# JoeyT1994/TensorNetworkQuantumSimulator.jl

Measured on AMD Instinct MI355X. Metric: two-site gates/sec at fixed chi (LxL TFIM Trotter layer), higher is better.
Workload: dtype c64 (ComplexF32; Gram/eigen steps in f64; the chi = 32 plane products as exact bf16 x 3 splits with f32 accumulation, TNQS_NO_BF16X3=1 for f32 matrix instructions)

## Files before the change

### include/tnqs_debug.h

```cpp
#ifndef TNQS_DEBUG_H
#define TNQS_DEBUG_H
#include <stdint.h>
#include "tnqs.h"
#ifdef __cplusplus
extern "C" {
#endif
int tnqs_dbg_jacobi(int dtype, int m, int n, void* A_inout, void* V_out, int* sweeps_out);
int tnqs_dbg_theta_svd_pre(int m, int n, int nq, void* A_inout, const void* Q, void* V_out, int* sweeps_out, int copies, int reps, double* ms_out, double* phase_us_out ,
                           int cap );
int tnqs_dbg_time_jacobi_f32(int m, int n, const void* A, int copies, int reps, double* ms_out, int* sweeps_out);
int tnqs_dbg_chol(int n, const void* G, void* L_out, void* W_out, int* fail_out, double tau);
int tnqs_dbg_fiber_gemm(int dtype, int D, int PA, int K, int PB, int Do, int No, const void* in, const void* X, void* out,
                        double* norm2_out, int use_mfma);
int tnqs_dbg_gram(int dtype, int D, int PA, int K, int PB, const void* X, const void* Y, void* out, int acc64, int use_mfma);
int tnqs_dbg_gram_fused(int PA, int K, int PB, const void* X, const void* Y, const void* M, void* out);
int tnqs_dbg_gauge_gram(int z, const int* chi, int bleg, const void* X, const void* M, void* out);
int tnqs_dbg_pair(int C0, int NMID, int NHI, const void* in, const void* Mx, const void* My, void* out);
int tnqs_dbg_pair_legs(int d, int z, const int* chi, int lx, int ly, const void* in, const void* Mx, const void* My, void* out);
int tnqs_dbg_pair_gram(int d, int z, const int* chi, int lx, int ly, const void* X, const void* Y, const void* M, void* out);
int tnqs_dbg_pair_gram2(int d, int z, const int* chi, int lx, int ly, const void* X, const void* Y, const void* Mx, const void* My, void* out_y, void* out_x);
int tnqs_dbg_bench_plane(int which, int nsites, int lx, int ly, int reps, double* ms);
#define TNQS_DBG_ROUTE_X3 1
#define TNQS_DBG_ROUTE_F32 2
#define TNQS_DBG_ROUTE_F64 3
#define TNQS_DBG_ROUTE_F64_SHARED 4
#define TNQS_DBG_ROUTE_HALF_LINES 5
#define TNQS_DBG_ROUTE_WHOLE_LINES 6
#define TNQS_DBG_ROUTE_SMALL_SCALAR 7
#define TNQS_DBG_ROUTE_SMALL_MFMA16 8
int tnqs_dbg_rowgemm(int D, int K, int nitems, const int* PA, const int* PB, const int* No, const void* in, const void* X, void* out, double* norm2_out,
                     int tpw, int* route_out);
int tnqs_dbg_gram_mfma(int nitems, const int* shape, const void* X, const void* Y, void* out, int nchunks, int* route_out);
int tnqs_dbg_pair16(int d, int nitems, const int* z, const int* chi, const int* lx, const int* ly, const void* in, const void* M, void* out, int spw, int* route_out);
int tnqs_dbg_pair_gram2x16(int d, int nitems, const int* z, const int* chi, const int* lx, const int* ly, const int* both, const void* X, const void* Y, const void* M,
                           void* out_y, void* out_x, int spw);
int tnqs_dbg_svd_tall(int nitems, const int* m, const int* n, void* A, int* chol_fail, int* polished, int* sweeps);
int tnqs_dbg_small_site(int nitems, const int* d, const int* z, const int* chi, const int* jo, const void* psi, const void* M, const int* present, int form,
                        const void* old_msg, const int* has_old, int normalize, void* out, void* new_msg, double* diff_out, int* route_out);
int tnqs_dbg_msg_finalize(int dtype, int nitems, const int* chi, const int* nchunks, const void* partials, const void* old_msg, const int* has_old, int normalize,
                          void* new_msg, double* diff_out);
int tnqs_dbg_default_sequence(tnqs_handle h, int* src, int* dst, int cap, int* n_out);
int tnqs_dbg_default_sequence_graph(int nv, int ne, const int32_t* esrc, const int32_t* edst, int* src, int* dst, int* level, int cap, int* n_out);
int tnqs_dbg_gate_schedule(int nv, int ne, const int32_t* esrc, const int32_t* edst, int ngates, const int32_t* nverts, const int32_t* verts, int update_cache,
                           int* step_of_gate, int* step_is_bp, int cap, int* nsteps_out);
#ifdef __cplusplus
}
#endif
#endif
```

### profiles/plane_bench.py

```python
import ctypes as C
import os
import sys

here = os.path.dirname(os.path.abspath(__file__))
lib = C.CDLL(os.path.join(here, "..", "tensornetworkquantumsimulator.jl_amd", "libtnqs_hip.so"))
lib.tnqs_dbg_bench_plane.argtypes = [C.c_int, C.c_int, C.c_int, C.c_int, C.c_int, C.POINTER(C.c_double)]
nsites = int(sys.argv[1]) if len(sys.argv) > 1 else 100
reps = int(sys.argv[2]) if len(sys.argv) > 2 else 5
n = 2 * 32 ** 4
for which, name, flops in ((0, "pair", 2 * 8.0 * n * 32), (1, "pair_gram2", 4 * 8.0 * n * 32)):
    for lx, ly in ((0, 1), (0, 2), (0, 3), (1, 2), (1, 3), (2, 3)):
        ms = C.c_double(0)
        rc = lib.tnqs_dbg_bench_plane(which, nsites, lx, ly, reps, C.byref(ms))
        if rc != 0:
            print(name, (lx, ly), "rc", rc)
            continue
        print(f"{name:11s} legs ({lx},{ly})  {ms.value:8.3f} ms  {flops * nsites / ms.value / 1e9:7.1f} TFLOP/s")
```

### tensornetworkquantumsimulator.jl_amd/csrc/api.cpp

```cpp
#include <cmath>
#include <cstring>
#include <string>
#include "engine.hpp"

using namespace tnqs;

struct tnqs_state_s { State* s; };

static thread_local std::string g_err;

template <class F> static int guard(F&& f) {
    try { f(); return TNQS_OK; }
    catch (const Err& e) { g_err = e.what(); return e.code; }
    catch (const std::bad_alloc&) { g_err = "out of host memory"; return TNQS_ERR_HIP; }
    catch (const std::exception& e) { g_err = e.what(); return TNQS_ERR_INVALID; }
    catch (...) { g_err = "unknown error"; return TNQS_ERR_INVALID; }
}
static State* S(tnqs_handle h) { if (!h || !h->s) throw Err(TNQS_ERR_INVALID, "null handle"); return h->s; }

extern "C" {

int tnqs_version(void) { return 102; }
const char* tnqs_last_error(void) { return g_err.c_str(); }
int tnqs_device_count(int* count) {
// ... 138 lines not shown

int tnqs_profile_enable(tnqs_handle h, int on) { return guard([&] { S(h)->prof->on = on != 0; }); }
int tnqs_profile_get(tnqs_handle h, int cls, int64_t* launches, double* ms, double* bytes, double* flops) {
    return guard([&] {
        State* s = S(h);
        if (cls < 0 || cls >= TNQS_PROF_NCLASSES) throw Err(TNQS_ERR_INVALID, "profile_get: bad class");
        prof_collect(s);
        const ProfClass& pc = s->prof->cls[cls];
        if (launches) *launches = pc.launches;
        if (ms) *ms = pc.ms;
        if (bytes) *bytes = pc.bytes;
        if (flops) *flops = pc.flops;
    });
}
int tnqs_profile_reset(tnqs_handle h) {
    return guard([&] { State* s = S(h); prof_collect(s); for (auto& p : s->prof->cls) p = ProfClass{}; });
}

}

#include "../../include/tnqs_debug.h"
#include "kernels.hpp"
namespace tnqs { void dbg_default_sequence(const Graph& g, std::vector<int>& src, std::vector<int>& dst);
                 std::shared_ptr<Graph> dbg_make_graph(int nv, int ne, const int32_t* es, const int32_t* ed);
                 void dbg_default_sequence_graph(const Graph& g, std::vector<int>& src, std::vector<int>& dst, std::vector<int>& level);
                 void dbg_pair(int C0, int NMID, int NHI, const void* in, const void* Mx, const void* My, void* out);
                 void dbg_gram_fused(int PA, int K, int PB, const void* X, const void* Y, const void* M, void* out);
                 void dbg_gauge_gram(int z, const int* chi, int bleg, const void* X, const void* M, void* out);
                 void dbg_jacobi(int dtype, int m, int n, void* A, void* V, int* sweeps);
                 void dbg_chol(int n, const void* G, void* L, void* W, int* fail, double tau);
                 void dbg_theta_svd_pre(int m, int n, int nq, void* A, const void* Q, void* V, int* sweeps, int copies, int reps, double* ms, double* phase_us, int cap);
                 void dbg_time_jacobi_f32(int m, int n, const void* A, int copies, int reps, double* ms, int* sweeps);
                 void dbg_pair_legs(int d, int z, const int* chi, int lx, int ly, const void* in, const void* Mx, const void* My, void* out);
                 void dbg_pair_gram2(int d, int z, const int* chi, int lx, int ly, const void* X, const void* Y, const void* Mx, const void* My, void* out_y, void* out_x);
                 void dbg_bench_plane(int which, int nsites, int lx, int ly, int reps, double* ms);
                 void dbg_pair_gram(int d, int z, const int* chi, int lx, int ly, const void* X, const void* Y, const void* M, void* out);
                 void dbg_fiber_gemm(int dtype, int D, int PA, int K, int PB, int Do, int No, const void* in, const void* X, void* out, double* norm2, int use_mfma);
                 void dbg_gram(int dtype, int D, int PA, int K, int PB, const void* X, const void* Y, void* out, int acc64, int use_mfma);
                 void dbg_rowgemm(int D, int K, int nitems, const int* PA, const int* PB, const int* No, const void* in, const void* X, void* out, double* norm2, int tpw, int* route);
                 void dbg_gram_mfma(int nitems, const int* shape, const void* X, const void* Y, void* out, int nchunks, int* route);
                 void dbg_pair16(int d, int nitems, const int* z, const int* chi, const int* lx, const int* ly, const void* in, const void* M, void* out, int spw, int* route);
                 void dbg_pair_gram2x16(int d, int nitems, const int* z, const int* chi, const int* lx, const int* ly, const int* both, const void* X, const void* Y, const void* M,
                                        void* out_y, void* out_x, int spw);
                 void dbg_svd_tall(int nitems, const int* m, const int* n, void* A, int* chol_fail, int* polished, int* sweeps);
                 void dbg_small_site(int nitems, const int* d, const int* z, const int* chi, const int* jo, const void* psi, const void* M, const int* present, int form,
                                     const void* old_msg, const int* has_old, int normalize, void* out, void* new_msg, double* diff, int* route);
                 void dbg_msg_finalize(int dtype, int nitems, const int* chi, const int* nchunks, const void* partials, const void* old_msg, const int* has_old, int normalize,
                                       void* new_msg, double* diff); }
extern "C" {
int tnqs_dbg_default_sequence(tnqs_handle h, int* src, int* dst, int cap, int* n_out) {
    return guard([&] { std::vector<int> a, b; dbg_default_sequence(*S(h)->g, a, b); *n_out = (int)a.size();
                       for (int i = 0; i < (int)a.size() && i < cap; ++i) { src[i] = a[i]; dst[i] = b[i]; } });
}
int tnqs_dbg_default_sequence_graph(int nv, int ne, const int32_t* esrc, const int32_t* edst, int* src, int* dst, int* level, int cap, int* n_out) {
    return guard([&] { if (nv < 0 || ne < 0 || (ne > 0 && (!esrc || !edst)) || !n_out) throw Err(TNQS_ERR_INVALID, "tnqs_dbg_default_sequence_graph: bad arguments");
                       auto g = dbg_make_graph(nv, ne, esrc, edst); std::vector<int> a, b, l; dbg_default_sequence_graph(*g, a, b, l); *n_out = (int)a.size();
                       for (int i = 0; i < (int)a.size() && i < cap; ++i) { if (src) src[i] = a[i]; if (dst) dst[i] = b[i]; if (level) level[i] = l[i]; } });
}
int tnqs_dbg_gate_schedule(int nv, int ne, const int32_t* esrc, const int32_t* edst, int ngates, const int32_t* nverts, const int32_t* verts, int update_cache,
                           int* step_of_gate, int* step_is_bp, int cap, int* nsteps_out) {
    return guard([&] { if (nv < 0 || ne < 0 || (ne > 0 && (!esrc || !edst)) || ngates < 0 || (ngates > 0 && (!nverts || !verts)) || !nsteps_out) throw Err(TNQS_ERR_INVALID, "tnqs_dbg_gate_schedule: bad arguments");
                       for (int i = 0, o = 0; i < ngates; o += nverts[i], ++i) { if (nverts[i] < 1 || nverts[i] > 2) throw Err(TNQS_ERR_INVALID, "tnqs_dbg_gate_schedule: only one- and two-site gates");
                                                                                 for (int k = 0; k < nverts[i]; ++k) if (verts[o + k] < 0 || verts[o + k] >= nv) throw Err(TNQS_ERR_INVALID, "tnqs_dbg_gate_schedule: vertex out of range"); }
                       auto g = dbg_make_graph(nv, ne, esrc, edst); const GateSchedule steps = build_gate_schedule(*g, ngates, nverts, verts, update_cache != 0); *nsteps_out = (int)steps.size();
                       for (int k = 0; k < (int)steps.size(); ++k) { if (step_is_bp && k < cap) step_is_bp[k] = steps[k].is_bp ? 1 : 0; if (step_of_gate) for (int i = steps[k].begin; i < steps[k].end; ++i) step_of_gate[i] = k; } });
}
int tnqs_dbg_jacobi(int dtype, int m, int n, void* A, void* V, int* sweeps) { return guard([&] { dbg_jacobi(dtype, m, n, A, V, sweeps); }); }
int tnqs_dbg_theta_svd_pre(int m, int n, int nq, void* A, const void* Q, void* V, int* sweeps, int copies, int reps, double* ms, double* phase_us, int cap) { return guard([&] { dbg_theta_svd_pre(m, n, nq, A, Q, V, sweeps, copies, reps, ms, phase_us, cap); }); }
int tnqs_dbg_time_jacobi_f32(int m, int n, const void* A, int copies, int reps, double* ms, int* sweeps) { return guard([&] { dbg_time_jacobi_f32(m, n, A, copies, reps, ms, sweeps); }); }
int tnqs_dbg_chol(int n, const void* G, void* L, void* W, int* fail, double tau) { return guard([&] { dbg_chol(n, G, L, W, fail, tau); }); }
int tnqs_dbg_fiber_gemm(int dtype, int D, int PA, int K, int PB, int Do, int No, const void* in, const void* X, void* out, double* norm2, int use_mfma) {
    return guard([&] { dbg_fiber_gemm(dtype, D, PA, K, PB, Do, No, in, X, out, norm2, use_mfma); });
}
int tnqs_dbg_pair(int C0, int NMID, int NHI, const void* in, const void* Mx, const void* My, void* out) { return guard([&] { dbg_pair(C0, NMID, NHI, in, Mx, My, out); }); }
int tnqs_dbg_pair_legs(int d, int z, const int* chi, int lx, int ly, const void* in, const void* Mx, const void* My, void* out) { return guard([&] { dbg_pair_legs(d, z, chi, lx, ly, in, Mx, My, out); }); }
int tnqs_dbg_pair_gram2(int d, int z, const int* chi, int lx, int ly, const void* X, const void* Y, const void* Mx, const void* My, void* out_y, void* out_x) {
    return guard([&] { dbg_pair_gram2(d, z, chi, lx, ly, X, Y, Mx, My, out_y, out_x); });
}
int tnqs_dbg_bench_plane(int which, int nsites, int lx, int ly, int reps, double* ms) { return guard([&] { dbg_bench_plane(which, nsites, lx, ly, reps, ms); }); }
int tnqs_dbg_pair_gram(int d, int z, const int* chi, int lx, int ly, const void* X, const void* Y, const void* M, void* out) { return guard([&] { dbg_pair_gram(d, z, chi, lx, ly, X, Y, M, out); }); }
int tnqs_dbg_gram_fused(int PA, int K, int PB, const void* X, const void* Y, const void* M, void* out) { return guard([&] { dbg_gram_fused(PA, K, PB, X, Y, M, out); }); }
int tnqs_dbg_gauge_gram(int z, const int* chi, int bleg, const void* X, const void* M, void* out) { return guard([&] { dbg_gauge_gram(z, chi, bleg, X, M, out); }); }
int tnqs_dbg_gram(int dtype, int D, int PA, int K, int PB, const void* X, const void* Y, void* out, int acc64, int use_mfma) {
    return guard([&] { dbg_gram(dtype, D, PA, K, PB, X, Y, out, acc64, use_mfma); });
}
int tnqs_dbg_rowgemm(int D, int K, int nitems, const int* PA, const int* PB, const int* No, const void* in, const void* X, void* out, double* norm2_out, int tpw, int* route_out) {
    return guard([&] { dbg_rowgemm(D, K, nitems, PA, PB, No, in, X, out, norm2_out, tpw, route_out); });
}
int tnqs_dbg_gram_mfma(int nitems, const int* shape, const void* X, const void* Y, void* out, int nchunks, int* route_out) {
    return guard([&] { dbg_gram_mfma(nitems, shape, X, Y, out, nchunks, route_out); });
}
int tnqs_dbg_pair16(int d, int nitems, const int* z, const int* chi, const int* lx, const int* ly, const void* in, const void* M, void* out, int spw, int* route_out) {
    return guard([&] { dbg_pair16(d, nitems, z, chi, lx, ly, in, M, out, spw, route_out); });
}
int tnqs_dbg_pair_gram2x16(int d, int nitems, const int* z, const int* chi, const int* lx, const int* ly, const int* both, const void* X, const void* Y, const void* M,
                           void* out_y, void* out_x, int spw) {
    return guard([&] { dbg_pair_gram2x16(d, nitems, z, chi, lx, ly, both, X, Y, M, out_y, out_x, spw); });
}
int tnqs_dbg_svd_tall(int nitems, const int* m, const int* n, void* A, int* chol_fail, int* polished, int* sweeps) {
    return guard([&] { dbg_svd_tall(nitems, m, n, A, chol_fail, polished, sweeps); });
}
int tnqs_dbg_small_site(int nitems, const int* d, const int* z, const int* chi, const int* jo, const void* psi, const void* M, const int* present, int form,
                        const void* old_msg, const int* has_old, int normalize, void* out, void* new_msg, double* diff_out, int* route_out) {
    return guard([&] { dbg_small_site(nitems, d, z, chi, jo, psi, M, present, form, old_msg, has_old, normalize, out, new_msg, diff_out, route_out); });
}
int tnqs_dbg_msg_finalize(int dtype, int nitems, const int* chi, const int* nchunks, const void* partials, const void* old_msg, const int* has_old, int normalize,
                          void* new_msg, double* diff_out) {
    return guard([&] { dbg_msg_finalize(dtype, nitems, chi, nchunks, partials, old_msg, has_old, normalize, new_msg, diff_out); });
// ... 3 lines not shown
```

### tensornetworkquantumsimulator.jl_amd/csrc/debug.cpp

```cpp
#include <cstdio>
#include <cstring>
#include <cstdlib>
#include <vector>
#include <algorithm>
#include <memory>
#include <string>
#include "engine.hpp"
#include "kernels.hpp"
#include "launch_util.hpp"
#include "../../include/tnqs_debug.h"

namespace tnqs {
#define HIPCHK(x) hipchk((x), #x)
struct DBuf { void* p = nullptr; explicit DBuf(size_t n) { HIPCHK(hipMalloc(&p, n ? n : 1)); } ~DBuf() { (void)hipFree(p); }
              void up(const void* h, size_t n) { HIPCHK(hipMemcpy(p, h, n, hipMemcpyHostToDevice)); } void down(void* h, size_t n) { HIPCHK(hipMemcpy(h, p, n, hipMemcpyDeviceToHost)); } };
static void need_gpu() { int n = 0; if (hipGetDeviceCount(&n) != hipSuccess || n <= 0) throw Err(TNQS_ERR_HIP, "no HIP device available"); }

void dbg_jacobi(int dtype, int m, int n, void* A, void* V, int* sweeps) {
    need_gpu();
    if (m < 1 || n < 1 || m > 256 || n > 256) throw Err(TNQS_ERR_INVALID, "dbg_jacobi: 1 <= m, n <= 256");
    size_t esz = dtype == TNQS_C64 ? 8 : 16;
    DBuf dA((size_t)m * n * esz), dV((size_t)n * n * esz), dS(4), dI(sizeof(JacobiItem));
    dA.up(A, (size_t)m * n * esz);
    if (dtype == TNQS_C64) launch_identity<float>(nullptr, dV.p, n); else launch_identity<double>(nullptr, dV.p, n);
// ... 152 lines not shown
}
void dbg_pair(int C0, int NMID, int NHI, const void* in, const void* Mx, const void* My, void* out) {
    need_gpu();
    if (C0 % 16) throw Err(TNQS_ERR_INVALID, "dbg_pair: C0 % 16 != 0");
    size_t n = (size_t)C0 * 32 * NMID * 32 * NHI;
    DBuf dIn(n * 8), dOut(n * 8), dX(32 * 32 * 8), dY(32 * 32 * 8), dI(sizeof(PairItem));
    dIn.up(in, n * 8); dX.up(Mx, 32 * 32 * 8); dY.up(My, 32 * 32 * 8);
    HIPCHK(hipMemset(dOut.p, 0xff, n * 8));
    PairItem it{}; it.in = dIn.p; it.out = dOut.p; it.Mx = dX.p; it.My = dY.p;
    it.g.cstr = 2; it.g.sx = C0; it.g.sy = (long long)C0 * 32 * NMID; it.g.n0 = C0 / 16; it.g.t0 = 16; it.g.n1 = NMID; it.g.t1 = (long long)C0 * 32;
    it.g.n2 = NHI; it.g.t2 = (long long)C0 * 32 * NMID * 32;
    const int wgs = plan_pair(&it, 1, 3);
    dI.up(&it, sizeof(it));
    launch_mfma_pair(nullptr, (const PairItem*)dI.p, 1, wgs);
    HIPCHK(hipDeviceSynchronize());
    dOut.down(out, n * 8);
}
void dbg_pair_legs(int d, int z, const int* chi, int lx, int ly, const void* in, const void* Mx, const void* My, void* out) {
    need_gpu();
    PairItem it{};
    if (!pair_geometry(d, z, chi, lx, ly, it.g)) throw Err(TNQS_ERR_UNSUPPORTED, "dbg_pair_legs: shape not covered by the pair kernel");
    size_t n = d; for (int i = 0; i < z; ++i) n *= chi[i];
    DBuf dIn(n * 8), dOut(n * 8), dX(32 * 32 * 8), dY(32 * 32 * 8), dI(sizeof(PairItem));
    dIn.up(in, n * 8); dX.up(Mx, 32 * 32 * 8); dY.up(My, 32 * 32 * 8);
    HIPCHK(hipMemset(dOut.p, 0xff, n * 8));
    it.in = dIn.p; it.out = dOut.p; it.Mx = dX.p; it.My = dY.p;
    if ((size_t)it.g.n0 * it.g.n1 * it.g.n2 * 16 * 1024 != n) throw Err(TNQS_ERR_INVALID, "dbg_pair_legs: slice count");
    const int wgs = plan_pair(&it, 1, 3);
    dI.up(&it, sizeof(it));
    launch_mfma_pair(nullptr, (const PairItem*)dI.p, 1, wgs);
    HIPCHK(hipDeviceSynchronize());
    dOut.down(out, n * 8);
}
void dbg_pair_gram(int d, int z, const int* chi, int lx, int ly, const void* X, const void* Y, const void* M, void* out) {
    need_gpu();
    PairGramItem it{};
    if (!pair_geometry(d, z, chi, lx, ly, it.g)) throw Err(TNQS_ERR_UNSUPPORTED, "dbg_pair_gram: shape not covered by the pair kernel");
    size_t n = d; for (int i = 0; i < z; ++i) n *= chi[i];
    const bool x3 = mfma_use_x3();
    PairGram2Item one{}; one.g = it.g;
    const int nwg = x3 ? plan_x3_pair_gram1(&one, 1, nullptr, 3) : plan_pair_gram(&it, 1, nullptr, 3), npart = nwg;
    DBuf dX(n * 8), dY(n * 8), dM(32 * 32 * 8), dI(sizeof(PairGram2Item)), dR(sizeof(ReduceItem)), dP((size_t)npart * 1024 * 8), dO(1024 * 8);
    dX.up(X, n * 8); dY.up(Y, n * 8); dM.up(M, 32 * 32 * 8);
    it.X = dX.p; it.Y = dY.p; it.M = dM.p; it.partial = dP.p;
    if (x3) {
        one.X = it.X; one.Y = it.Y; one.Mx = it.M; one.partial_y = it.partial;
        dI.up(&one, sizeof(one));
        launch_x3_pair_gram1(nullptr, (const PairGram2Item*)dI.p, 1, nwg);
    } else {
        dI.up(&it, sizeof(it));
        launch_mfma_pair_gram(nullptr, (const PairGramItem*)dI.p, 1, nwg);
    }
    ReduceItem ri{dP.p, dO.p, 1024, npart, 0, 0}; dR.up(&ri, sizeof(ri));
    launch_reduce<float, float>(nullptr, (const ReduceItem*)dR.p, 1, 1024);
    HIPCHK(hipDeviceSynchronize());
    dO.down(out, 1024 * 8);
}
void dbg_pair_gram2(int d, int z, const int* chi, int lx, int ly, const void* X, const void* Y, const void* Mx, const void* My, void* out_y, void* out_x) {
    need_gpu();
    PairGram2Item it{};
    if (!pair_geometry(d, z, chi, lx, ly, it.g)) throw Err(TNQS_ERR_UNSUPPORTED, "dbg_pair_gram2: shape not covered");
    size_t n = d; for (int i = 0; i < z; ++i) n *= chi[i];
    const int nwg = plan_pair_gram2(&it, 1, nullptr, 3), npart = nwg;
    DBuf dX(n * 8), dY(n * 8), dMx(1024 * 8), dMy(1024 * 8), dI(sizeof(PairGram2Item)), dR(2 * sizeof(ReduceItem)), dP1((size_t)npart * 1024 * 8), dP2((size_t)npart * 1024 * 8), dO(2 * 1024 * 8);
    dX.up(X, n * 8); dY.up(Y, n * 8); dMx.up(Mx, 1024 * 8); dMy.up(My, 1024 * 8);
    it.X = dX.p; it.Y = dY.p; it.Mx = dMx.p; it.My = dMy.p; it.partial_y = dP1.p; it.partial_x = dP2.p;
// ... 475 lines not shown
```

### tensornetworkquantumsimulator.jl_amd/csrc/kernels_mfma.hip

```cpp
#include <cstdlib>
#include "kernels.hpp"
#include "mfma_common.hpp"
#include <type_traits>
#include "launch_util.hpp"

namespace tnqs {

template <int KB, int NB, int TR>
__global__ __launch_bounds__(256) void mfma_fiber_gemm_kernel(const FiberItem* __restrict__ items, int nitems,
                                                              double* __restrict__ norm_partials) {
    constexpr int KKP = 32 * KB, NNP = 32 * NB;
    constexpr int CP = (KKP > NNP ? KKP : NNP);
    constexpr int PT = CP + 1;
    constexpr int PX = KKP + 1;
    constexpr int RB = TR / 32;
    constexpr int NU = 8;
    static_assert(RB * NB == 4, "one (row block, column block) unit per wave");
    extern __shared__ __attribute__((aligned(16))) char smem[];
    float* At_re = reinterpret_cast<float*>(smem);
    float* At_im = At_re + TR * PT;
    float* Xt_re = At_im + TR * PT;
    float* Xt_im = Xt_re + NNP * PX;
    __shared__ double sh_red[4];
    const int tid = threadIdx.x;
// ... 662 lines not shown
                const int q = 4 * c4 + i;
                const float br = mxr[q], bi = mxi[q];
                if (q == 0) Y.template mac_bpre<true>(xc[i][0], xc[i][1], br, M3 ? bi - br : bi, M3 ? br + bi : -bi);
                else Y.template mac_bpre<false>(xc[i][0], xc[i][1], br, M3 ? bi - br : bi, M3 ? br + bi : -bi);
                if ((q & 1) == 0) { pre[q >> 1] = ldg4(in + nb + tstr * (q >> 1)); TNQS_PIN(); }
            }
#pragma unroll
            for (int i = 0; i < 4; ++i) xc[i] = xn[i];
        }
        CAcc32<M3> S;
#pragma unroll
        for (int r = 0; r < 16; ++r) {
            const float br = myr[r], bi = myi[r];
            if (r == 0) S.template mac_bpre<true>(Y.re(r), Y.im(r), br, M3 ? bi - br : bi, M3 ? br + bi : -bi);
            else S.template mac_bpre<false>(Y.re(r), Y.im(r), br, M3 ? bi - br : bi, M3 ? br + bi : -bi);
            if ((r & 1) == 0) { if (prev) store1(buf ^ 1, ob, r >> 1); TNQS_PIN(); }
        }
        S.finish();
#pragma unroll
        for (int r = 0; r < 16; ++r) { const int jx = (r & 3) + 8 * (r >> 2) + 4 * h; v2f v; v[0] = S.a[r]; v[1] = S.b[r]; P[ln * 33 + jx] = v; }
        if (more) commit(buf ^ 1);
        lds_barrier();
    }
    if (s_begin < s_end) {
        const int buf = (s_end - 1 - s_begin) & 1;
        const long long ob = pair_slice_base(g, s_end - 1) + toff;
#pragma unroll
        for (int j = 0; j < 8; ++j) store1(buf, ob, j);
    }
    #undef TNQS_PIN
}
static int pair_slices(const PairGeom& g) { return g.n0 * g.n1 * g.n2; }
int plan_pair(PairItem* it, int n, int spw) {
    if (spw <= 0) {
        double tot = 0; for (int i = 0; i < n; ++i) tot += pair_slices(it[i].g); spw = 16; while (spw > 1 && 2.0 * tot / spw < 1024.0) spw >>= 1;
#ifdef TNQS_EXPERIMENTS
        static const int forced = [] { const char* e = std::getenv("TNQS_PAIR_SPW"); return e ? std::atoi(e) : 0; }();
        if (forced > 0) spw = forced;
#endif
    }
    return lay_out(it, n, &PairItem::slice_begin, nullptr, [&](PairItem& p) { p.spw = spw; const int np = (pair_slices(p.g) + spw - 1) / spw; return 16 * ((np + 7) / 8); });
}
void launch_mfma_pair(hipStream_t s, const PairItem* d_items, int nitems, int total_wgs) {
    if (total_wgs <= 0) return;
    if (mfma_use_x3()) { launch_x3_pair(s, d_items, nitems, total_wgs); return; }
    const size_t lds = (size_t)16 * (32 * 33 + 4) * 2 * sizeof(float);
    set_max_dynamic_lds((const void*)mfma_pair_kernel<true>, lds); hipLaunchKernelGGL(mfma_pair_kernel<true>, dim3(total_wgs), dim3(512), lds, s, d_items, nitems);
    TNQS_CHECK_LAUNCH();
}

__global__ __launch_bounds__(512) void mfma_pair_gram_kernel(const PairGramItem* __restrict__ items, int nitems, int xcd) {
    constexpr int PS = 32 * 33 + 1;
    extern __shared__ __attribute__((aligned(16))) char smem[];
    v2f* L = reinterpret_cast<v2f*>(smem);
    const int tid = threadIdx.x, lane = tid & 63, w = tid >> 6, ln = lane & 31, h = lane >> 5;
    int lo = 0, hi_ = nitems - 1;
    const int gw = xcd_remap(blockIdx.x, gridDim.x, xcd);
    while (lo < hi_) { int mid = (lo + hi_ + 1) >> 1; if (items[mid].wg_begin <= gw) lo = mid; else hi_ = mid - 1; }
    const PairGramItem it = items[lo];
    const PairGeom g = it.g;
    const int nslices = g.n0 * g.n1 * g.n2;
    const int lw = gw - it.wg_begin;
    const int s_begin = lw * it.spw, s_end = min(nslices, s_begin + it.spw);
    const cf* __restrict__ Xg = reinterpret_cast<const cf*>(it.X);
    const cf* __restrict__ Yg = reinterpret_cast<const cf*>(it.Y);
    const cf* __restrict__ Mg = reinterpret_cast<const cf*>(it.M);
    float mr[16], mi[16];
#pragma unroll
    for (int q = 0; q < 16; ++q) { cf v = Mg[(q + 16 * h) + 32 * ln]; mr[q] = v.re; mi[q] = v.im; }
    v16f Or, Oi;
#pragma unroll
    for (int r = 0; r < 16; ++r) { Or[r] = 0.f; Oi[r] = 0.f; }
    const int f = tid & 7, sg0 = tid >> 3;
    const long long sx = g.sx, sy = g.sy, fo = (long long)f * g.cstr;
// ... 495 lines not shown
```

### tensornetworkquantumsimulator.jl_amd/csrc/kernels_x3.hip

```cpp
#include <cstdlib>
#include <type_traits>
#include "kernels.hpp"
#include "mfma_common.hpp"
#include "launch_util.hpp"
#include "x3_common.hpp"

namespace tnqs {

__device__ __forceinline__ long long x3_slice_base(const PairGeom& g, int sl) {
    int a0 = sl % g.n0; int r1 = sl / g.n0; int a1 = r1 % g.n1; int a2 = r1 / g.n1;
    return (long long)a0 * g.t0 + (long long)a1 * g.t1 + (long long)a2 * g.t2;
}

template <int MODE, bool SINGLE = false>
__global__ __launch_bounds__(512) __attribute__((amdgpu_waves_per_eu(2, 2))) void x3_pair_gram2_kernel(const PairGram2Item* __restrict__ items, int nitems) {
    constexpr int P = 34;
    constexpr int PS = 32 * P + 2;
    #define TNQS_PIN() __builtin_amdgcn_sched_barrier(0x2 | 0x4)
    extern __shared__ __attribute__((aligned(16))) char smem[];
    v2f* L = reinterpret_cast<v2f*>(smem);
    const int tid = threadIdx.x, lane = tid & 63, w = tid >> 6, ln = lane & 31, h = lane >> 5;
    int lo = 0, hi_ = nitems - 1;
    const int gw = blockIdx.x;
    while (lo < hi_) { int mid = (lo + hi_ + 1) >> 1; if (items[mid].wg_begin <= gw) lo = mid; else hi_ = mid - 1; }
// ... 162 lines not shown
}
#undef TNQS_PIN
int x3_pair_gram2_group() { return 16; }
int plan_x3_pair_gram1(PairGram2Item* it, int n, int* nwg, int spw) {
    auto slices = [](const PairGram2Item& p) { return p.g.n0 * p.g.n1 * p.g.n2; };
    if (spw <= 0) { double tot = 0; for (int i = 0; i < n; ++i) tot += (double)slices(it[i]); spw = 16; while (spw > 1 && 2.0 * tot / spw < 1024.0) spw >>= 1; }
    return lay_out(it, n, &PairGram2Item::wg_begin, nwg, [&](PairGram2Item& p) { p.spw = spw; const int np = (slices(p) + spw - 1) / spw; return 16 * ((np + 7) / 8); });
}
void launch_x3_pair_gram1(hipStream_t s, const PairGram2Item* d_items, int nitems, int total_wgs) {
    if (total_wgs <= 0) return;
    const size_t lds = (size_t)16 * (32 * 34 + 2) * 2 * sizeof(float);
    set_max_dynamic_lds((const void*)x3_pair_gram2_kernel<0, true>, lds);
    hipLaunchKernelGGL((x3_pair_gram2_kernel<0, true>), dim3(total_wgs), dim3(512), lds, s, d_items, nitems);
    TNQS_CHECK_LAUNCH();
}
void launch_x3_pair_gram2(hipStream_t s, const PairGram2Item* d_items, int nitems, int total_wgs) {
    if (total_wgs <= 0) return;
    const size_t lds = (size_t)16 * (32 * 34 + 2) * 2 * sizeof(float);
#ifdef TNQS_EXPERIMENTS
    static const int mode = [] { const char* e = std::getenv("TNQS_X3_MODE"); return e ? std::atoi(e) : 0; }();
    #define TNQS_X3_LAUNCH(M) { set_max_dynamic_lds((const void*)x3_pair_gram2_kernel<M>, lds); hipLaunchKernelGGL(x3_pair_gram2_kernel<M>, dim3(total_wgs), dim3(512), lds, s, d_items, nitems); }
    if (mode == 1) TNQS_X3_LAUNCH(1) else if (mode == 2) TNQS_X3_LAUNCH(2) else if (mode == 3) TNQS_X3_LAUNCH(3) else if (mode == 4) TNQS_X3_LAUNCH(4) else if (mode == 5) TNQS_X3_LAUNCH(5) else TNQS_X3_LAUNCH(0)
    #undef TNQS_X3_LAUNCH
#else
    set_max_dynamic_lds((const void*)x3_pair_gram2_kernel<0>, lds);
    hipLaunchKernelGGL(x3_pair_gram2_kernel<0>, dim3(total_wgs), dim3(512), lds, s, d_items, nitems);
#endif
    TNQS_CHECK_LAUNCH();
}

__global__ __launch_bounds__(512) __attribute__((amdgpu_waves_per_eu(2, 2))) void x3_pair_kernel(const PairItem* __restrict__ items, int nitems) {
    constexpr int P = 34;
    constexpr int PS = 32 * P + 2;
    constexpr int BUF = 8 * PS;
    extern __shared__ __attribute__((aligned(16))) char smem[];
    v2f* L = reinterpret_cast<v2f*>(smem);
    const int tid = threadIdx.x, lane = tid & 63, w = tid >> 6, ln = lane & 31, h = lane >> 5;
    int lo = 0, hi_ = nitems - 1;
    const int gw = blockIdx.x;
    while (lo < hi_) { int mid = (lo + hi_ + 1) >> 1; if (items[mid].slice_begin <= gw) lo = mid; else hi_ = mid - 1; }
    const PairItem it = items[lo];
    const PairGeom g = it.g;
    const int nslices = g.n0 * g.n1 * g.n2;
    const int lw = gw - it.slice_begin;
    const int half = (lw >> 3) & 1, pw = ((lw >> 4) << 3) | (lw & 7);
    const int s_begin = pw * it.spw, s_end = min(nslices, s_begin + it.spw);
    const cf* __restrict__ in = reinterpret_cast<const cf*>(it.in);
    cf* __restrict__ out = reinterpret_cast<cf*>(it.out);
    P3 Mxr[2], Mxi[2];
    u4* const MyL = reinterpret_cast<u4*>(L + 16 * PS) + lane;
    {
        const cf* __restrict__ Mx = reinterpret_cast<const cf*>(it.Mx) + 32 * ln; const cf* __restrict__ My = reinterpret_cast<const cf*>(it.My) + 32 * ln;
#pragma unroll
        for (int n = 0; n < 2; ++n) {
            float xr[8], xi[8];
#pragma unroll
            for (int e = 0; e < 8; e += 2) { const v4f v = ldg4(Mx + 16 * n + 8 * h + e); xr[e] = v[0]; xi[e] = v[1]; xr[e + 1] = v[2]; xi[e + 1] = v[3]; }
            Mxr[n] = split8(xr); Mxi[n] = split8(xi);
#pragma unroll
            for (int e = 0; e < 8; e += 2) { const v4f v = ldg4(My + 4 * h + 16 * n + 8 * (e >> 2) + (e & 3)); xr[e] = v[0]; xi[e] = v[1]; xr[e + 1] = v[2]; xi[e + 1] = v[3]; }
            const P3 yr_ = split8(xr), yi_ = split8(xi);
            if (w == 0) { MyL[(6 * n + 0) * 64] = yr_.h; MyL[(6 * n + 1) * 64] = yr_.m; MyL[(6 * n + 2) * 64] = yr_.l; MyL[(6 * n + 3) * 64] = yi_.h; MyL[(6 * n + 4) * 64] = yi_.m; MyL[(6 * n + 5) * 64] = yi_.l; }
        }
    }
    const int f4 = tid & 3, sg0 = tid >> 2;
    const int ix0 = sg0 & 31, iy0 = sg0 >> 5;
    const long long toff = (long long)(4 * half + f4) * g.cstr + g.sx * ix0 + g.sy * iy0, tstr = 4 * g.sy;
    v2f* const lbase = L + (2 * f4) * PS + iy0 * P + ix0;
    v4f preA[8], preB[8];
    #define TNQS_PIN() __builtin_amdgcn_sched_barrier(0x2 | 0x4)
    auto commit = [&](int buf, const v4f (&pre)[8]) {
#pragma unroll
        for (int j = 0; j < 8; ++j) {
            v2f* p0 = lbase + buf * BUF + 4 * P * j;
            v2f a; a[0] = pre[j][0]; a[1] = pre[j][1]; v2f b; b[0] = pre[j][2]; b[1] = pre[j][3];
            p0[0] = a; p0[PS] = b;
        }
    };
    auto store1 = [&](int buf, long long ob, int j) {
        const v2f* p0 = lbase + buf * BUF + 4 * P * j;
        const v2f a = p0[0], c = p0[PS];
        v4f v; v[0] = a[0]; v[1] = a[1]; v[2] = c[0]; v[3] = c[1];
        stg4(out + ob + tstr * j, v);
    };
    if (s_begin < s_end) {
        const long long b = x3_slice_base(g, s_begin) + toff;
#pragma unroll
        for (int j = 0; j < 8; ++j) preB[j] = ldg4(in + b + tstr * j);
        const long long b1 = x3_slice_base(g, s_begin + 1 < s_end ? s_begin + 1 : s_begin) + toff;
#pragma unroll
        for (int j = 0; j < 8; ++j) preA[j] = ldg4(in + b1 + tstr * j);
        commit(0, preB);
    }
    lds_barrier();
    auto phase = [&](int sl, int buf, const v4f (&cur)[8], v4f (&nxt)[8]) {
        const bool more = sl + 1 < s_end, prev = sl > s_begin;
        const long long nb = x3_slice_base(g, sl + 2 < s_end ? sl + 2 : sl) + toff;
        const long long ob = x3_slice_base(g, prev ? sl - 1 : sl) + toff;
        v2f* Pw = L + buf * BUF + w * PS;
        v16f Yr, Yi;
#pragma unroll
        for (int n = 0; n < 2; ++n) {
            float ar[8], ai[8];
            const v4f* a = reinterpret_cast<const v4f*>(Pw + ln * P + 16 * n + 8 * h);
#pragma unroll
            for (int q = 0; q < 4; ++q) { const v4f v = a[q]; ar[2 * q] = v[0]; ai[2 * q] = v[1]; ar[2 * q + 1] = v[2]; ai[2 * q + 1] = v[3]; }
#pragma unroll
            for (int j = 0; j < 4; ++j) nxt[4 * n + j] = ldg4(in + nb + tstr * (4 * n + j));
            TNQS_PIN();
            const P3 sr = split8(ar), si = split8(ai), nsi = neg(si);
            if (n == 0) mac6x2<true>(Yr, sr, Mxr[n], Yi, sr, Mxi[n]); else mac6x2<false>(Yr, sr, Mxr[n], Yi, sr, Mxi[n]);
            mac6x2<false>(Yr, nsi, Mxi[n], Yi, si, Mxr[n]);
        }
        v16f Sr, Si;
#pragma unroll
        for (int n = 0; n < 2; ++n) {
            float yr[8], yi[8];
#pragma unroll
            for (int e = 0; e < 8; ++e) { yr[e] = Yr[8 * n + e]; yi[e] = Yi[8 * n + e]; }
            const P3 pr = split8(yr), pi = split8(yi), npi = neg(pi);
            if (prev) {
#pragma unroll
                for (int j = 0; j < 4; ++j) store1(buf ^ 1, ob, 4 * n + j);
            }
            P3 myr, myi;
            myr.h = MyL[(6 * n + 0) * 64]; myr.m = MyL[(6 * n + 1) * 64]; myr.l = MyL[(6 * n + 2) * 64]; myi.h = MyL[(6 * n + 3) * 64]; myi.m = MyL[(6 * n + 4) * 64]; myi.l = MyL[(6 * n + 5) * 64];
            TNQS_PIN();
            if (n == 0) mac6x2<true>(Sr, pr, myr, Si, pr, myi); else mac6x2<false>(Sr, pr, myr, Si, pr, myi);
            mac6x2<false>(Sr, npi, myi, Si, pi, myr);
        }
        TNQS_PIN();
#pragma unroll
        for (int r = 0; r < 16; r += 2) { const int jx = (r & 3) + 8 * (r >> 2) + 4 * h; v4f v; v[0] = Sr[r]; v[1] = Si[r]; v[2] = Sr[r + 1]; v[3] = Si[r + 1]; *reinterpret_cast<v4f*>(Pw + ln * P + jx) = v; }
        if (more) commit(buf ^ 1, cur);
        lds_barrier();
    };
    for (int sl = s_begin; sl < s_end; sl += 2) {
        phase(sl, 0, preA, preB);
        if (sl + 1 < s_end) phase(sl + 1, 1, preB, preA);
    }
    if (s_begin < s_end) {
        const int buf = (s_end - 1 - s_begin) & 1;
        const long long ob = x3_slice_base(g, s_end - 1) + toff;
#pragma unroll
        for (int j = 0; j < 8; ++j) store1(buf, ob, j);
    }
    #undef TNQS_PIN
}
void launch_x3_pair(hipStream_t s, const PairItem* d_items, int nitems, int total_wgs) {
    if (total_wgs <= 0) return;
    const size_t lds = (size_t)16 * (32 * 34 + 2) * 2 * sizeof(float) + 12 * 64 * 16;
    set_max_dynamic_lds((const void*)x3_pair_kernel, lds);
    hipLaunchKernelGGL(x3_pair_kernel, dim3(total_wgs), dim3(512), lds, s, d_items, nitems);
    TNQS_CHECK_LAUNCH();
}

template <int D>
__global__ __launch_bounds__(256, 2) void x3_rowgemm64_kernel(const FiberItem* __restrict__ items, int nitems, double* __restrict__ norm_partials) {
    constexpr int KK = 64;
    extern __shared__ __attribute__((aligned(16))) char smem[];
    u4* const Xl = reinterpret_cast<u4*>(smem);
    __shared__ double sh_red[4];
    const int tid = threadIdx.x, lane = tid & 63, w = tid >> 6, ln = lane & 31, h = lane >> 5;
    int lo = 0, hi = nitems - 1;
    const int gw = blockIdx.x;
    while (lo < hi) { int mid = (lo + hi + 1) >> 1; if (items[mid].tile_begin <= gw) lo = mid; else hi = mid - 1; }
    const FiberItem it = items[lo];
    const int K = it.K, No = it.No, NN = it.Do * No;
    const long long PA = it.PA;
    const int ntiles = it.nta * it.ntb;
    const int t_begin = (gw - it.tile_begin) * it.tpw, t_end = min(ntiles, t_begin + it.tpw);
    const cf* __restrict__ in = reinterpret_cast<const cf*>(it.in);
    const cf* __restrict__ X = reinterpret_cast<const cf*>(it.X);
    cf* __restrict__ out = reinterpret_cast<cf*>(it.out);
    for (int e = tid; e < 4 * 2 * 64; e += 256) {
        const int l = e & 63, nb = (e >> 6) & 1, n = e >> 7;
        const int nn = 32 * nb + (l & 31), kk0 = 16 * n + 8 * (l >> 5);
        float xr[8], xi[8];
// ... 259 lines not shown
```

Baseline: 6631.

## Process whole 16-plane slices per workgroup in x3 pair kernel

The x3 pair kernel previously split each slice into two half-workgroups of 8 planes, using double-buffered LDS that overlapped loads and stores with compute. Each workgroup now owns all 16 planes of a slice, with each wave doing two planes. It uses a single LDS buffer, stores the finished slice, commits the prefetched next slice and issues loads two slices ahead between barriers. The planner drops the half-slice workgroup grouping when x3 is active, which halves the workgroup count per slice and changes the spw heuristic. The aim is to cut redundant matrix setup per workgroup and improve load/store coalescing, at the cost of less compute/memory overlap within the slice loop.

Result: slower. 6534 (-1.5%).

```diff
diff --git a/include/tnqs_debug.h b/include/tnqs_debug.h
--- a/include/tnqs_debug.h
+++ b/include/tnqs_debug.h
@@ -17,6 +17,7 @@
 int tnqs_dbg_gauge_gram(int z, const int* chi, int bleg, const void* X, const void* M, void* out);
 int tnqs_dbg_pair(int C0, int NMID, int NHI, const void* in, const void* Mx, const void* My, void* out);
 int tnqs_dbg_pair_legs(int d, int z, const int* chi, int lx, int ly, const void* in, const void* Mx, const void* My, void* out);
+int tnqs_dbg_pair_legs_batch(int d, int nitems, const int* z, const int* chi, const int* lx, const int* ly, const void* in, const void* M, void* out, int spw);
 int tnqs_dbg_pair_gram(int d, int z, const int* chi, int lx, int ly, const void* X, const void* Y, const void* M, void* out);
 int tnqs_dbg_pair_gram2(int d, int z, const int* chi, int lx, int ly, const void* X, const void* Y, const void* Mx, const void* My, void* out_y, void* out_x);
 int tnqs_dbg_bench_plane(int which, int nsites, int lx, int ly, int reps, double* ms);
diff --git a/profiles/plane_bench.py b/profiles/plane_bench.py
--- a/profiles/plane_bench.py
+++ b/profiles/plane_bench.py
@@ -7,12 +7,16 @@
 lib.tnqs_dbg_bench_plane.argtypes = [C.c_int, C.c_int, C.c_int, C.c_int, C.c_int, C.POINTER(C.c_double)]
 nsites = int(sys.argv[1]) if len(sys.argv) > 1 else 100
 reps = int(sys.argv[2]) if len(sys.argv) > 2 else 5
+only = sys.argv[3] if len(sys.argv) > 3 else None
 n = 2 * 32 ** 4
 for which, name, flops in ((0, "pair", 2 * 8.0 * n * 32), (1, "pair_gram2", 4 * 8.0 * n * 32)):
+    if only and name != only:
+        continue
     for lx, ly in ((0, 1), (0, 2), (0, 3), (1, 2), (1, 3), (2, 3)):
         ms = C.c_double(0)
         rc = lib.tnqs_dbg_bench_plane(which, nsites, lx, ly, reps, C.byref(ms))
         if rc != 0:
             print(name, (lx, ly), "rc", rc)
             continue
-        print(f"{name:11s} legs ({lx},{ly})  {ms.value:8.3f} ms  {flops * nsites / ms.value / 1e9:7.1f} TFLOP/s")
+        tbs = f"  {2 * 8.0 * n * nsites / ms.value / 1e9:5.2f} TB/s" if which == 0 else ""
+        print(f"{name:11s} legs ({lx},{ly})  {ms.value:8.3f} ms  {flops * nsites / ms.value / 1e9:7.1f} TFLOP/s{tbs}")
diff --git a/tensornetworkquantumsimulator.jl_amd/csrc/api.cpp b/tensornetworkquantumsimulator.jl_amd/csrc/api.cpp
--- a/tensornetworkquantumsimulator.jl_amd/csrc/api.cpp
+++ b/tensornetworkquantumsimulator.jl_amd/csrc/api.cpp
@@ -194,6 +194,7 @@
                  void dbg_theta_svd_pre(int m, int n, int nq, void* A, const void* Q, void* V, int* sweeps, int copies, int reps, double* ms, double* phase_us, int cap);
                  void dbg_time_jacobi_f32(int m, int n, const void* A, int copies, int reps, double* ms, int* sweeps);
                  void dbg_pair_legs(int d, int z, const int* chi, int lx, int ly, const void* in, const void* Mx, const void* My, void* out);
+                 void dbg_pair_legs_batch(int d, int nitems, const int* z, const int* chi, const int* lx, const int* ly, const void* in, const void* M, void* out, int spw);
                  void dbg_pair_gram2(int d, int z, const int* chi, int lx, int ly, const void* X, const void* Y, const void* Mx, const void* My, void* out_y, void* out_x);
                  void dbg_bench_plane(int which, int nsites, int lx, int ly, int reps, double* ms);
                  void dbg_pair_gram(int d, int z, const int* chi, int lx, int ly, const void* X, const void* Y, const void* M, void* out);
@@ -236,6 +237,9 @@
 }
 int tnqs_dbg_pair(int C0, int NMID, int NHI, const void* in, const void* Mx, const void* My, void* out) { return guard([&] { dbg_pair(C0, NMID, NHI, in, Mx, My, out); }); }
 int tnqs_dbg_pair_legs(int d, int z, const int* chi, int lx, int ly, const void* in, const void* Mx, const void* My, void* out) { return guard([&] { dbg_pair_legs(d, z, chi, lx, ly, in, Mx, My, out); }); }
+int tnqs_dbg_pair_legs_batch(int d, int nitems, const int* z, const int* chi, const int* lx, const int* ly, const void* in, const void* M, void* out, int spw) {
+    return guard([&] { dbg_pair_legs_batch(d, nitems, z, chi, lx, ly, in, M, out, spw); });
+}
 int tnqs_dbg_pair_gram2(int d, int z, const int* chi, int lx, int ly, const void* X, const void* Y, const void* Mx, const void* My, void* out_y, void* out_x) {
     return guard([&] { dbg_pair_gram2(d, z, chi, lx, ly, X, Y, Mx, My, out_y, out_x); });
 }
diff --git a/tensornetworkquantumsimulator.jl_amd/csrc/debug.cpp b/tensornetworkquantumsimulator.jl_amd/csrc/debug.cpp
--- a/tensornetworkquantumsimulator.jl_amd/csrc/debug.cpp
+++ b/tensornetworkquantumsimulator.jl_amd/csrc/debug.cpp
@@ -208,6 +208,30 @@
     HIPCHK(hipDeviceSynchronize());
     dOut.down(out, n * 8);
 }
+void dbg_pair_legs_batch(int d, int nitems, const int* z, const int* chi, const int* lx, const int* ly, const void* in, const void* M, void* out, int spw) {
+    need_gpu();
+    if (nitems < 1 || !z || !chi || !lx || !ly || !in || !M || !out) throw Err(TNQS_ERR_INVALID, "dbg_pair_legs_batch: bad arguments");
+    std::vector<PairItem> items(nitems); std::vector<size_t> off(nitems + 1, 0);
+    for (int i = 0, c = 0; i < nitems; c += z[i], ++i) {
+        if (!pair_geometry(d, z[i], chi + c, lx[i], ly[i], items[i].g)) throw Err(TNQS_ERR_UNSUPPORTED, "dbg_pair_legs_batch: shape not covered by the pair kernel");
+        size_t n = d; for (int k = 0; k < z[i]; ++k) n *= chi[c + k];
+        if ((size_t)items[i].g.n0 * items[i].g.n1 * items[i].g.n2 * 16 * 1024 != n) throw Err(TNQS_ERR_INVALID, "dbg_pair_legs_batch: slice count");
+        off[i + 1] = off[i] + n;
+    }
+    const size_t n = off[nitems];
+    DBuf dIn(n * 8), dOut(n * 8), dM((size_t)nitems * 2048 * 8), dI(sizeof(PairItem) * nitems);
+    dIn.up(in, n * 8); dM.up(M, (size_t)nitems * 2048 * 8);
+    HIPCHK(hipMemset(dOut.p, 0xff, n * 8));
+    for (int i = 0; i < nitems; ++i) {
+        PairItem& it = items[i];
+        it.in = (char*)dIn.p + off[i] * 8; it.out = (char*)dOut.p + off[i] * 8; it.Mx = (char*)dM.p + (size_t)i * 2048 * 8; it.My = (char*)it.Mx + 1024 * 8;
+    }
+    const int wgs = plan_pair(items.data(), nitems, spw);
+    dI.up(items.data(), sizeof(PairItem) * nitems);
+    launch_mfma_pair(nullptr, (const PairItem*)dI.p, nitems, wgs);
+    HIPCHK(hipDeviceSynchronize());
+    dOut.down(out, n * 8);
+}
 void dbg_pair_gram(int d, int z, const int* chi, int lx, int ly, const void* X, const void* Y, const void* M, void* out) {
     need_gpu();
     PairGramItem it{};
diff --git a/tensornetworkquantumsimulator.jl_amd/csrc/kernels_mfma.hip b/tensornetworkquantumsimulator.jl_amd/csrc/kernels_mfma.hip
--- a/tensornetworkquantumsimulator.jl_amd/csrc/kernels_mfma.hip
+++ b/tensornetworkquantumsimulator.jl_amd/csrc/kernels_mfma.hip
@@ -718,14 +718,15 @@
 }
 static int pair_slices(const PairGeom& g) { return g.n0 * g.n1 * g.n2; }
 int plan_pair(PairItem* it, int n, int spw) {
+    const bool whole = mfma_use_x3();
     if (spw <= 0) {
-        double tot = 0; for (int i = 0; i < n; ++i) tot += pair_slices(it[i].g); spw = 16; while (spw > 1 && 2.0 * tot / spw < 1024.0) spw >>= 1;
+        double tot = 0; for (int i = 0; i < n; ++i) tot += pair_slices(it[i].g); spw = 16; while (spw > 1 && (whole ? 1.0 : 2.0) * tot / spw < 1024.0) spw >>= 1;
 #ifdef TNQS_EXPERIMENTS
         static const int forced = [] { const char* e = std::getenv("TNQS_PAIR_SPW"); return e ? std::atoi(e) : 0; }();
         if (forced > 0) spw = forced;
 #endif
     }
-    return lay_out(it, n, &PairItem::slice_begin, nullptr, [&](PairItem& p) { p.spw = spw; const int np = (pair_slices(p.g) + spw - 1) / spw; return 16 * ((np + 7) / 8); });
+    return lay_out(it, n, &PairItem::slice_begin, nullptr, [&](PairItem& p) { p.spw = spw; const int np = (pair_slices(p.g) + spw - 1) / spw; return whole ? np : 16 * ((np + 7) / 8); });
 }
 void launch_mfma_pair(hipStream_t s, const PairItem* d_items, int nitems, int total_wgs) {
     if (total_wgs <= 0) return;
diff --git a/tensornetworkquantumsimulator.jl_amd/csrc/kernels_x3.hip b/tensornetworkquantumsimulator.jl_amd/csrc/kernels_x3.hip
--- a/tensornetworkquantumsimulator.jl_amd/csrc/kernels_x3.hip
+++ b/tensornetworkquantumsimulator.jl_amd/csrc/kernels_x3.hip
@@ -218,7 +218,6 @@
 __global__ __launch_bounds__(512) __attribute__((amdgpu_waves_per_eu(2, 2))) void x3_pair_kernel(const PairItem* __restrict__ items, int nitems) {
     constexpr int P = 34;
     constexpr int PS = 32 * P + 2;
-    constexpr int BUF = 8 * PS;
     extern __shared__ __attribute__((aligned(16))) char smem[];
     v2f* L = reinterpret_cast<v2f*>(smem);
     const int tid = threadIdx.x, lane = tid & 63, w = tid >> 6, ln = lane & 31, h = lane >> 5;
@@ -229,8 +228,7 @@
     const PairGeom g = it.g;
     const int nslices = g.n0 * g.n1 * g.n2;
     const int lw = gw - it.slice_begin;
-    const int half = (lw >> 3) & 1, pw = ((lw >> 4) << 3) | (lw & 7);
-    const int s_begin = pw * it.spw, s_end = min(nslices, s_begin + it.spw);
+    const int s_begin = lw * it.spw, s_end = min(nslices, s_begin + it.spw);
     const cf* __restrict__ in = reinterpret_cast<const cf*>(it.in);
     cf* __restrict__ out = reinterpret_cast<cf*>(it.out);
     P3 Mxr[2], Mxi[2];
@@ -249,41 +247,43 @@
             if (w == 0) { MyL[(6 * n + 0) * 64] = yr_.h; MyL[(6 * n + 1) * 64] = yr_.m; MyL[(6 * n + 2) * 64] = yr_.l; MyL[(6 * n + 3) * 64] = yi_.h; MyL[(6 * n + 4) * 64] = yi_.m; MyL[(6 * n + 5) * 64] = yi_.l; }
         }
     }
-    const int f4 = tid & 3, sg0 = tid >> 2;
+    const int f8 = tid & 7, sg0 = tid >> 3;
     const int ix0 = sg0 & 31, iy0 = sg0 >> 5;
-    const long long toff = (long long)(4 * half + f4) * g.cstr + g.sx * ix0 + g.sy * iy0, tstr = 4 * g.sy;
-    v2f* const lbase = L + (2 * f4) * PS + iy0 * P + ix0;
+    const long long toff = (long long)f8 * g.cstr + g.sx * ix0 + g.sy * iy0, tstr = 2 * g.sy;
+    v2f* const lbase = L + (2 * f8) * PS + iy0 * P + ix0;
     v4f preA[8], preB[8];
     #define TNQS_PIN() __builtin_amdgcn_sched_barrier(0x2 | 0x4)
-    auto commit = [&](int buf, const v4f (&pre)[8]) {
+    auto load8 = [&](v4f (&pre)[8], long long b, int j0) {
+#pragma unroll
+        for (int j = 0; j < 8; ++j) pre[j] = ldg4(in + b + tstr * (j0 + j));
+    };
+    auto commit = [&](const v4f (&pre)[8], int j0) {
 #pragma unroll
         for (int j = 0; j < 8; ++j) {
-            v2f* p0 = lbase + buf * BUF + 4 * P * j;
+            v2f* p0 = lbase + 2 * P * (j0 + j);
             v2f a; a[0] = pre[j][0]; a[1] = pre[j][1]; v2f b; b[0] = pre[j][2]; b[1] = pre[j][3];
             p0[0] = a; p0[PS] = b;
         }
     };
-    auto store1 = [&](int buf, long long ob, int j) {
-        const v2f* p0 = lbase + buf * BUF + 4 * P * j;
-        const v2f a = p0[0], c = p0[PS];
-        v4f v; v[0] = a[0]; v[1] = a[1]; v[2] = c[0]; v[3] = c[1];
-        stg4(out + ob + tstr * j, v);
+    auto store8 = [&](long long ob, int j0) {
+        v4f v[8];
+#pragma unroll
+        for (int j = 0; j < 8; ++j) {
+            const v2f* p0 = lbase + 2 * P * (j0 + j);
+            const v2f a = p0[0], c = p0[PS];
+            v[j][0] = a[0]; v[j][1] = a[1]; v[j][2] = c[0]; v[j][3] = c[1];
+        }
+#pragma unroll
+        for (int j = 0; j < 8; ++j) stg4(out + ob + tstr * (j0 + j), v[j]);
     };
     if (s_begin < s_end) {
         const long long b = x3_slice_base(g, s_begin) + toff;
-#pragma unroll
-        for (int j = 0; j < 8; ++j) preB[j] = ldg4(in + b + tstr * j);
-        const long long b1 = x3_slice_base(g, s_begin + 1 < s_end ? s_begin + 1 : s_begin) + toff;
-#pragma unroll
-        for (int j = 0; j < 8; ++j) preA[j] = ldg4(in + b1 + tstr * j);
-        commit(0, preB);
+        load8(preA, b, 0); load8(preB, b, 8);
+        commit(preA, 0); commit(preB, 8);
+        if (s_begin + 1 < s_end) { const long long b1 = x3_slice_base(g, s_begin + 1) + toff; load8(preA, b1, 0); load8(preB, b1, 8); }
     }
     lds_barrier();
-    auto phase = [&](int sl, int buf, const v4f (&cur)[8], v4f (&nxt)[8]) {
-        const bool more = sl + 1 < s_end, prev = sl > s_begin;
-        const long long nb = x3_slice_base(g, sl + 2 < s_end ? sl + 2 : sl) + toff;
-        const long long ob = x3_slice_base(g, prev ? sl - 1 : sl) + toff;
-        v2f* Pw = L + buf * BUF + w * PS;
+    auto plane = [&](v2f* Pw) {
         v16f Yr, Yi;
 #pragma unroll
         for (int n = 0; n < 2; ++n) {
@@ -291,8 +291,6 @@
             const v4f* a = reinterpret_cast<const v4f*>(Pw + ln * P + 16 * n + 8 * h);
 #pragma unroll
             for (int q = 0; q < 4; ++q) { const v4f v = a[q]; ar[2 * q] = v[0]; ai[2 * q] = v[1]; ar[2 * q + 1] = v[2]; ai[2 * q + 1] = v[3]; }
-#pragma unroll
-            for (int j = 0; j < 4; ++j) nxt[4 * n + j] = ldg4(in + nb + tstr * (4 * n + j));
             TNQS_PIN();
             const P3 sr = split8(ar), si = split8(ai), nsi = neg(si);
             if (n == 0) mac6x2<true>(Yr, sr, Mxr[n], Yi, sr, Mxi[n]); else mac6x2<false>(Yr, sr, Mxr[n], Yi, sr, Mxi[n]);
@@ -305,10 +303,6 @@
 #pragma unroll
             for (int e = 0; e < 8; ++e) { yr[e] = Yr[8 * n + e]; yi[e] = Yi[8 * n + e]; }
             const P3 pr = split8(yr), pi = split8(yi), npi = neg(pi);
-            if (prev) {
-#pragma unroll
-                for (int j = 0; j < 4; ++j) store1(buf ^ 1, ob, 4 * n + j);
-            }
             P3 myr, myi;
             myr.h = MyL[(6 * n + 0) * 64]; myr.m = MyL[(6 * n + 1) * 64]; myr.l = MyL[(6 * n + 2) * 64]; myi.h = MyL[(6 * n + 3) * 64]; myi.m = MyL[(6 * n + 4) * 64]; myi.l = MyL[(6 * n + 5) * 64];
             TNQS_PIN();
@@ -318,18 +312,19 @@
         TNQS_PIN();
 #pragma unroll
         for (int r = 0; r < 16; r += 2) { const int jx = (r & 3) + 8 * (r >> 2) + 4 * h; v4f v; v[0] = Sr[r]; v[1] = Si[r]; v[2] = Sr[r + 1]; v[3] = Si[r + 1]; *reinterpret_cast<v4f*>(Pw + ln * P + jx) = v; }
-        if (more) commit(buf ^ 1, cur);
+    };
+    for (int sl = s_begin; sl < s_end; ++sl) {
+        plane(L + w * PS);
+        plane(L + (w + 8) * PS);
         lds_barrier();
-    };
-    for (int sl = s_begin; sl < s_end; sl += 2) {
-        phase(sl, 0, preA, preB);
-        if (sl + 1 < s_end) phase(sl + 1, 1, preB, preA);
-    }
-    if (s_begin < s_end) {
-        const int buf = (s_end - 1 - s_begin) & 1;
-        const long long ob = x3_slice_base(g, s_end - 1) + toff;
-#pragma unroll
-        for (int j = 0; j < 8; ++j) store1(buf, ob, j);
+        const long long ob = x3_slice_base(g, sl) + toff;
+        const bool more = sl + 1 < s_end;
+        store8(ob, 0);
+        if (more) commit(preA, 0);
+        store8(ob, 8);
+        if (more) commit(preB, 8);
+        if (sl + 2 < s_end) { const long long nb = x3_slice_base(g, sl + 2) + toff; load8(preA, nb, 0); load8(preB, nb, 8); }
+        lds_barrier();
     }
     #undef TNQS_PIN
 }
```
